# facebook/zstd

Hardware: NVIDIA H100
Metric: compress GB/s (input) at level 1 (higher is better)
Workload: dtype u8

## Files before the change

zstd_b200/csrc/zb_api.cu:

```cuda
#include <cuda_runtime.h>
#include <stdio.h>
#include <stdlib.h>
#include <string.h>
#include <vector>
#include <memory>
#include <mutex>
#include <thread>
#include <new>
#include <time.h>
#include "../../include/zstd_b200.h"
#include "zb_common.h"
#include "zb_kernels.h"

static inline u32 hb32(u32 v) { return 31u - (u32)__builtin_clz(v); }

typedef struct { u32 windowLog, chainLog, hashLog, searchLog, minMatch, targetLength, strategy; } ZbCParams;
struct Row { u8 W, C, H, S, L, TL, strat; };
static const Row kRows[4][5] = {
    { {19,12,13,1,6,1,1}, {19,13,14,1,7,0,1}, {20,15,16,1,6,0,1}, {21,16,17,1,5,0,2}, {21,18,18,1,5,0,2} },
    { {18,12,13,1,5,1,1}, {18,13,14,1,6,0,1}, {18,14,14,1,5,0,2}, {18,16,16,1,4,0,2}, {18,16,16,1,4,0,2} },
    { {17,12,12,1,5,1,1}, {17,12,13,1,6,0,1}, {17,13,15,1,5,0,1}, {17,15,16,2,5,0,2}, {17,17,17,2,4,0,2} },
    { {14,12,13,1,5,1,1}, {14,14,15,1,5,0,1}, {14,14,15,1,4,0,1}, {14,14,15,2,4,0,2}, {14,14,15,2,4,0,2} },
};

// ... 93 lines not shown
        size_t const c = want < 2 * cap ? 2 * cap : want;
        T* q = NULL; bool pin = !pageable;
        if (pin && cudaMallocHost((void**)&q, c * sizeof(T)) != cudaSuccess) { cudaGetLastError(); pin = false; }
        if (!pin) q = (T*)malloc(c * sizeof(T));
        if (n) memcpy(q, p, n * sizeof(T));
        size_t const keep = n;
        release(); p = q; n = keep; cap = c; pinned = pin;
    }
    void push_back(const T& v) { if (n == cap) reserve(cap ? 2 * cap : 64); p[n++] = v; }
    void resize(size_t m) { reserve(m); if (m > n) memset((void*)(p + n), 0, (m - n) * sizeof(T)); n = m; }
    void clear() { n = 0; }
    size_t size() const { return n; }
    T* data() { return p; }
    const T* data() const { return p; }
    T& back() { return p[n - 1]; }
    T& operator[](size_t i) { return p[i]; }
    const T& operator[](size_t i) const { return p[i]; }
};
struct ZbLdmFrame { u32 frame; ZbLdmParams prm; u64 matchBase; u64 prefix; };
struct ZbPlan { ZbVec<ZbBlock> blocks; ZbVec<ZbChunk> chunks; ZbVec<ZbFrame> frames; std::vector<ZbGroup> groups; ZbStrides sd; bool unsupported;
                std::vector<ZbLdmFrame> ldm; u64 ldmMatches;
                u64 frameBytes, frameBlocks; u32 frameMaxBlock;
                void reset() { blocks.clear(); chunks.clear(); frames.clear(); groups.clear(); unsupported = false; ldm.clear(); ldmMatches = 0;
                               frameBytes = frameBlocks = 0; frameMaxBlock = 0; } };

enum { EV_START, EV_K0, EV_K1, EV_K2, EV_K3, EV_MID, EV_KEND, EV_END, EV_PHASES };

struct ZSTD_CCtx_s {
    int device;
    int bindDevice;
    ZbStream stream;
    ZbDevBuf<ZbChunk> d_chunks;
    ZbDevBuf<u8> d_work;
    u32 devWaveBlocks;
    ZbStream waveStream[ZB_WAVE_SLOTS_MAX + 1];
    u32 waveSlots;
    u32 hostWaveSlots;
    u32 hostWaveBlocks;
    ZbDevBuf<ZbBlock> d_blocks; ZbDevBuf<ZbFrame> d_frames;
    ZbDevBuf<u64> d_outOffsets, d_frameSizes;
    ZbDevBuf<u64> d_totals;
    ZbHostBuf<u64> h_totals;
    ZbDevBuf<u8> d_in, d_out;
    std::unique_ptr<ZSTD_CDict, ZbCDictFree> callDict;
    ZbEvents ev;
    ZbEvents evH2D, evStitch, evSize, evD2H;
    ZSTDB200_stats stats;
    int advLevel, advChecksum, advNoDictID;
    int advLdm;
    u32 advLdmPrm[4];
    ZbDevBuf<u64> d_ldmMatch, d_ldmFirst; ZbDevBuf<u32> d_ldmCnt; ZbDevBuf<u8> d_ldmScratch;
    std::unique_ptr<ZSTD_CDict, ZbCDictFree> advLocalDict;
    const ZSTD_CDict* advRefCDict;
    const u8* advPrefix; size_t advPrefixSize; bool advPrefixOnDevice;
    ZbDevBuf<u8> d_prefix;
    ZbPlan plan;
    u8* stIn; size_t stInSize, stInCap;
    u8* stOut; size_t stOutSize, stOutPos, stOutCap;
    int stFrames;
    int advDelims;
    ZbDevBuf<ZSTD_Sequence> d_seqIn;
    ZbDevBuf<u8> d_seqTile, d_seqBlk; ZbDevBuf<u64> d_seqCtrl;
    ZbOrder order; ZbEvents evStage, evJoin;
    ZbPlan asyncPlan;
    ZbHostBuf<u8> stage[ZSTDB200_ASYNC_SLOTS]; bool stageBusy[ZSTDB200_ASYNC_SLOTS]; u32 stageNext;
};
// ... 21 lines not shown
    c->device = -1;
    c->bindDevice = zb_contextDevice();
    c->advLevel = 3;
    c->asyncPlan.blocks.pageable = c->asyncPlan.chunks.pageable = c->asyncPlan.frames.pageable = true;
    {   const char* s = getenv("ZSTDB200_SERIAL"); const char* w = getenv("ZSTDB200_WAVE_BLOCKS");
        c->devWaveBlocks = (s && atoi(s)) ? 0u : (w ? (u32)atoi(w) : 1024u);
        const char* n = getenv("ZSTDB200_WAVE_SLOTS"); const char* h = getenv("ZSTDB200_HOST_WAVE_BLOCKS");
        c->waveSlots = n ? (u32)atoi(n) : ZB_WAVE_SLOTS_DEFAULT;
        c->hostWaveSlots = n ? (u32)atoi(n) : ZB_HOST_WAVE_SLOTS_DEFAULT;
        if (c->waveSlots < 1u) c->waveSlots = 1u;
        if (c->waveSlots > ZB_WAVE_SLOTS_MAX) c->waveSlots = ZB_WAVE_SLOTS_MAX;
        if (c->hostWaveSlots < 1u) c->hostWaveSlots = 1u;
        if (c->hostWaveSlots > ZB_WAVE_SLOTS_MAX) c->hostWaveSlots = ZB_WAVE_SLOTS_MAX;
        c->hostWaveBlocks = (h && atoi(h) > 0) ? (u32)atoi(h) : ZB_HOST_WAVE_BLOCKS; }
    return c;
}

static size_t zb_ctxInit(ZSTD_CCtx* c)
{
    if (c->device >= 0) { CK(cudaSetDevice(c->device)); return 0; }
    int n = 0;
    if (cudaGetDeviceCount(&n) != cudaSuccess || n == 0) { cudaGetLastError(); return ZB_ERR(ZB_error_GENERIC); }
    int dev = c->bindDevice;
    if (dev < 0) { if (cudaGetDevice(&dev) != cudaSuccess) dev = 0; }
    CK(cudaSetDevice(dev));
    ZbStream st; ZbEvents ev, evStage, evJoin; ZbOrder order;
    TRY(st.ensure());
    TRY(ev.ensure(EV_PHASES, true));
    TRY(order.create()); TRY(evStage.ensure(ZSTDB200_ASYNC_SLOTS, false)); TRY(evJoin.ensure(ZB_WAVE_SLOTS_MAX, false));
    static ZbdFseCTable defaults[3]; static std::once_flag once;
    std::call_once(once, [] { zb_buildDefaultTables(defaults); });
    CK(zb_upload_default_tables(defaults, st));
    CK(cudaStreamSynchronize(st));
    c->stream = std::move(st); c->ev = std::move(ev);
    c->order = std::move(order); c->evStage = std::move(evStage); c->evJoin = std::move(evJoin);
    c->device = dev;
    return 0;
}

extern "C" size_t ZSTD_freeCCtx(ZSTD_CCtx* c)
{
    if (!c) return 0;
    free(c->stIn); free(c->stOut);
    return zb_deleteOnDevice(c, &c->order);
}

static size_t zb_ensureDesc(ZSTD_CCtx* c, size_t nbBlocks, size_t nbFrames, size_t nbWaves, size_t nbChunks)
{
    TRY(c->d_chunks.ensure(nbChunks));
    TRY(c->d_blocks.ensure(nbBlocks)); TRY(c->d_outOffsets.ensure(nbBlocks + 1));
    TRY(c->d_frames.ensure(nbFrames)); TRY(c->d_frameSizes.ensure(nbFrames));
    TRY(c->d_totals.ensure(nbWaves)); TRY(c->h_totals.ensure(nbWaves));
    return 0;
}

struct ZbCall {
    void* dst; size_t dstCapacity; const void* src;
    const size_t* frameOffsets; const size_t* frameSizes; size_t nbFrames;
    const ZSTD_CDict* cdict;
    int level; size_t* cSizes;
    bool deviceMemory; cudaStream_t stream;
    bool checksum, noDictID;
    u64 partBegin = 0, partEnd = ~0ull;
    const u32* ldm = nullptr;
    const u8* prefix = nullptr; u64 prefixSize = 0; bool prefixOnDevice = false;
    unsigned long long* result = nullptr; unsigned long long* d_cSizes = nullptr;
// ... 171 lines not shown
    }
    size_t const nbBlocks = P.blocks.size();
    TRY(c->d_ldmMatch.ensure(P.ldmMatches));
    TRY(c->d_ldmFirst.ensure(nbBlocks));
    TRY(c->d_ldmCnt.ensure(nbBlocks));
    TRY(c->d_ldmScratch.ensure(scratch));
    return 0;
}
static size_t zb_runLdm(ZSTD_CCtx* c, const ZbPlan& P, const u8* d_src, const u8* d_prefix, cudaStream_t stream, unsigned* launches)
{
    for (size_t i = 0; i < P.ldm.size(); i++) {
        ZbLdmFrame const& lf = P.ldm[i];
        ZbFrame const& fr = P.frames[lf.frame];
        CK(zb_launch_ldm(d_prefix, lf.prefix, d_src + fr.srcOff, fr.srcSize, &lf.prm, c->d_ldmScratch, fr.nbBlocks, lf.matchBase, c->d_ldmMatch,
                         c->d_ldmFirst + fr.firstBlock, c->d_ldmCnt + fr.firstBlock, stream));
        *launches += 4u + 3u * ((lf.prm.hashLog - lf.prm.bucketSizeLog + 7u) / 8u);
        if (lf.prefix >= lf.prm.minMatch && fr.srcSize >= lf.prm.minMatch) *launches += 1u;
    }
    return 0;
}

static size_t zb_runBlocks(ZSTD_CCtx* c, const ZbPlan& P, const u8* d_src, const u8* d_dictEnd, const ZbDictEntropy* d_de, u32 b0, u32 b1, u32 c0, u32 c1,
                           const ZbWorkRows& rows, cudaStream_t stream, bool timed, unsigned* launches)
{
    for (int phase = 0; phase < 3; phase++) {
        for (size_t g = 0; g < P.groups.size(); g++) {
            ZbGroup const& G = P.groups[g];
            u32 const lo = G.b0 > b0 ? G.b0 : b0, hi = G.b1 < b1 ? G.b1 : b1;
            u32 const clo = G.c0 > c0 ? G.c0 : c0, chi = G.c1 < c1 ? G.c1 : c1;
            if (lo >= hi) continue;
            ZbWorkRows const R = rows.at(lo - b0);
            if (phase == 0) {
                ZbLdmView lv; lv.match = c->d_ldmMatch; lv.first = c->d_ldmFirst + lo; lv.cnt = c->d_ldmCnt + lo;
                CK(zb_launch_match(d_src, d_dictEnd, d_dictEnd ? G.image : (const u32*)0, c->d_blocks + lo, hi - lo, c->d_chunks + clo, chi - clo, lo, &G.prm, &R,
                                   (timed && P.groups.size() == 1) ? c->ev[EV_MID] : (cudaEvent_t)0, stream, G.ldm ? &lv : nullptr));
                *launches += G.prm.strategy == 2 ? 4 : 3;
            } else if (phase == 1) {
                CK(zb_launch_literals(c->d_blocks + lo, hi - lo, &G.prm, &R.sd, d_de, R.lits, R.body, R.meta, stream));
                *launches += 1;
            } else {
                CK(zb_launch_sequences(d_src, c->d_blocks + lo, hi - lo, &G.prm, &R.sd, d_de, R.seqs, R.dist, R.body, R.meta, stream));
                *launches += 1;
            }
        }
        if (timed) CK(cudaEventRecord(c->ev[EV_K1 + phase], stream));
    }
    return 0;
}

static u64 zb_xxh64(const u8* p, size_t len)
{
    u64 const P1 = 0x9E3779B185EBCA87ull, P2 = 0xC2B2AE3D27D4EB4Full, P3 = 0x165667B19E3779F9ull, P4 = 0x85EBCA77C2B2AE63ull, P5 = 0x27D4EB2F165667C5ull;
    auto rotl = [](u64 x, int r) { return (x << r) | (x >> (64 - r)); };
    auto rd64 = [](const u8* q) { u64 v; memcpy(&v, q, 8); return v; };
    auto rd32 = [](const u8* q) { u32 v; memcpy(&v, q, 4); return v; };
    auto round = [&](u64 acc, u64 in) { return rotl(acc + in * P2, 31) * P1; };
    auto merge = [&](u64 acc, u64 v) { return (acc ^ round(0, v)) * P1 + P4; };
    const u8* const end = p + len;
    u64 h;
    if (len >= 32) {
        u64 v1 = P1 + P2, v2 = P2, v3 = 0, v4 = 0 - P1;
        const u8* const limit = end - 32;
        do { v1 = round(v1, rd64(p)); v2 = round(v2, rd64(p + 8)); v3 = round(v3, rd64(p + 16)); v4 = round(v4, rd64(p + 24)); p += 32; } while (p <= limit);
        h = rotl(v1, 1) + rotl(v2, 7) + rotl(v3, 12) + rotl(v4, 18);
        h = merge(h, v1); h = merge(h, v2); h = merge(h, v3); h = merge(h, v4);
    } else h = P5;
    h += (u64)len;
// ... 906 lines not shown
```

zstd_b200/csrc/zb_common.h:

```cpp
#ifndef ZB_COMMON_H
#define ZB_COMMON_H
#include <stdint.h>
#include <stddef.h>

typedef uint8_t  u8;
typedef uint16_t u16;
typedef uint32_t u32;
typedef uint64_t u64;

#define ZB_BLOCK_MAX     (128u << 10)
#define ZB_PRIME_BYTES   (128u << 10)
#define ZB_CHUNK_BLOCKS  4u
#define ZB_BATCH         1024u
#define ZB_TAG_BITS      11u
#define ZB_FAST_HASHLOG_MAX   14u
#ifndef ZB_DFAST_SHORT_MAX
#define ZB_DFAST_SHORT_MAX    28672u
#endif
#ifndef ZB_DFAST_LONGLOG_MAX
#define ZB_DFAST_LONGLOG_MAX  14u
#endif
#define ZB_FAR           0xFFFFu

#define ZB_BT_RAW 0
// ... 164 lines not shown

static inline bool zb_isErr(size_t c) { return c > ZB_ERR(ZB_error_maxCode); }

#define CK(x) do { cudaError_t e_ = (x); if (e_ != cudaSuccess) { \
    if (getenv("ZSTDB200_DEBUG")) fprintf(stderr, "zstd_b200: CUDA error %s at %s:%d\n", cudaGetErrorString(e_), __FILE__, __LINE__); \
    cudaGetLastError(); return ZB_ERR(e_ == cudaErrorMemoryAllocation ? ZB_error_memory_allocation : ZB_error_GENERIC); } } while (0)
#define TRY(x) do { size_t const e_ = (x); if (zb_isErr(e_)) return e_; } while (0)

inline thread_local bool zb_noAlloc = false;

template <typename T, bool Pinned> struct ZbBuf {
    T* p = nullptr; size_t cap = 0;
    ZbBuf() = default;
    ZbBuf(const ZbBuf&) = delete; ZbBuf& operator=(const ZbBuf&) = delete;
    ~ZbBuf() { release(); }
    void release() { if (p) { if (Pinned) cudaFreeHost(p); else cudaFree(p); } p = nullptr; cap = 0; }
    size_t ensure(size_t need, size_t headroom = 0) {
        if (need <= cap) return 0;
        if (zb_noAlloc) return ZB_ERR(ZB_error_stage_wrong);
        release();
        size_t const bytes = (need + headroom) * sizeof(T);
        CK(Pinned ? cudaMallocHost((void**)&p, bytes) : cudaMalloc((void**)&p, bytes));
        cap = need + headroom;
        return 0;
    }
    operator T*() const { return p; }
};
template <typename T> using ZbDevBuf = ZbBuf<T, false>;
template <typename T> using ZbHostBuf = ZbBuf<T, true>;

enum ZbWorkKind { ZB_WORK_FAST, ZB_WORK_DFAST, ZB_WORK_SEQUENCES };
struct ZbWorkRows {
    ZbStrides sd;
    ZbBlockMeta* meta; u64* seqs; u8* lits; u8* body; u16* dist; u32* far; u16* dist2; u32* far2; ZbSegMeta* segmeta;
    ZbWorkRows at(size_t row) const {
        ZbWorkRows r = *this;
        auto down = [row](auto*& p, size_t stride) { if (p) p += row * stride; };
        down(r.meta, 1); down(r.seqs, sd.seq); down(r.lits, sd.lit); down(r.body, sd.body);
        down(r.dist, sd.dist); down(r.far, sd.dist); down(r.dist2, sd.dist); down(r.far2, sd.dist); down(r.segmeta, zb_segsPerRow(sd));
        return r;
    }
};
static inline size_t zb_workLayout(u8* base, size_t rows, ZbWorkKind kind, const ZbStrides& sd, ZbWorkRows* out)
{
    bool const match = kind != ZB_WORK_SEQUENCES;
    if (3ull * sd.state > sd.dist) return ZB_ERR(ZB_error_GENERIC);
    if (match && ((u64)sd.seq * 8u > (u64)sd.dist * 4u || ((u64)sd.seq + 1u) * 4u > (u64)sd.dist * 2u)) return ZB_ERR(ZB_error_GENERIC);
    ZbWorkRows w = {};
    w.sd = sd;
    size_t const align = (size_t)2 << 20;
    size_t bytes = 0;
    auto place = [&](auto*& p, size_t n) {
        if (base) p = reinterpret_cast<std::remove_reference_t<decltype(p)>>(base + bytes);
        bytes = (bytes + n * sizeof(*p) + 256u + align - 1u) & ~(align - 1u);
    };
    place(w.meta, rows); place(w.seqs, rows * sd.seq); place(w.lits, rows * sd.lit); place(w.body, rows * sd.body);
    place(w.dist, rows * sd.dist);
    if (match) { place(w.far, rows * sd.dist); place(w.segmeta, rows * zb_segsPerRow(sd)); }
    if (kind == ZB_WORK_DFAST) { place(w.dist2, rows * sd.dist); place(w.far2, rows * sd.dist); }
    if (base) *out = w;
    return bytes;
}

struct ZbStream {
    cudaStream_t s = nullptr;
    ZbStream() = default;
    ZbStream& operator=(ZbStream&& o) { std::swap(s, o.s); return *this; }
    ~ZbStream() { if (s) cudaStreamDestroy(s); }
    size_t ensure() {
        if (s) return 0;
        if (zb_noAlloc) return ZB_ERR(ZB_error_stage_wrong);
        CK(cudaStreamCreateWithFlags(&s, cudaStreamNonBlocking));
        return 0;
    }
    operator cudaStream_t() const { return s; }
};

struct ZbEvents {
    std::vector<cudaEvent_t> ev; bool timed = false;
    ZbEvents() = default;
    ZbEvents& operator=(ZbEvents&& o) { ev.swap(o.ev); std::swap(timed, o.timed); return *this; }
    ~ZbEvents() { release(); }
    void release() { for (cudaEvent_t e : ev) cudaEventDestroy(e); ev.clear(); }
    size_t ensure(size_t n, bool timing) {
        if (n <= ev.size() && timing == timed) return 0;
        if (zb_noAlloc) return ZB_ERR(ZB_error_stage_wrong);
        release();
        timed = timing;
        while (ev.size() < n) {
            cudaEvent_t e;
            CK(cudaEventCreateWithFlags(&e, timing ? cudaEventDefault : cudaEventDisableTiming));
// ... 54 lines not shown
```

zstd_b200/csrc/zb_kernels.h:

```cpp
#ifndef ZB_KERNELS_H
#define ZB_KERNELS_H
#include <cuda_runtime.h>
#include "zb_common.h"

#ifdef __cplusplus
extern "C" {
#endif

cudaError_t zb_launch_dict_image(const u8* d_dictEnd, const ZbChunk* d_dictChunk, const ZbParams* prm, u32* d_image, cudaStream_t stream);
cudaError_t zb_launch_match(const u8* d_src, const u8* d_dictEnd, const u32* d_image, const ZbBlock* d_blocks, u32 nbBlocks,
                            const ZbChunk* d_chunks, u32 nbChunks, u32 slotFirstBlock, const ZbParams* prm, const ZbWorkRows* rows,
                            cudaEvent_t evMid, cudaStream_t stream, const ZbLdmView* ldm = nullptr);

size_t zb_ldm_scratch_bytes(u64 P, u64 n, const ZbLdmParams* prm);
cudaError_t zb_launch_ldm(const u8* d_prefix, u64 P, const u8* d_frame, u64 n, const ZbLdmParams* prm, void* d_scratch, u32 nbBlocks,
                          u64 matchBase, u64* d_match, u64* d_ldmFirst, u32* d_ldmCnt, cudaStream_t stream);

cudaError_t zb_launch_seq_partition(const void* d_seqs, u32 n, int expl, u64* d_tileLen, u32* d_tileEnds, u64* d_ctrl, cudaStream_t stream);
cudaError_t zb_launch_seq_place(const void* d_seqs, u32 n, int expl, const u64* d_tileLen, const u32* d_tileEnds,
                                u64 srcSize, u64 window, u64 dictContent, u32 blockMax, u32 nbBlocks,
                                u64* d_blockEnd, u32* d_blockSeq, u32* d_blockFirst, u64* d_blockFirstPos, u64* d_ctrl, cudaStream_t stream);
cudaError_t zb_launch_seq_blocks(const u64* d_blockEnd, const u32* d_blockSeq, u32 nbBlocks, u32 blockMax, u32 dictFlag,
                                 ZbBlock* d_blocks, u32* d_blockFirst, u64* d_blockFirstPos, u64* d_ctrl, cudaStream_t stream);
cudaError_t zb_launch_seq_convert(const u8* d_src, const ZbBlock* d_blocks, u32 nbBlocks, const u32* d_blockFirst, const u64* d_blockFirstPos,
                                  const void* d_seqs, u32 n, const ZbParams* prm, const ZbWorkRows* rows, cudaStream_t stream);

void zb_buildDefaultTables(ZbdFseCTable* out3);
cudaError_t zb_upload_default_tables(const ZbdFseCTable* host3, cudaStream_t stream);

size_t zb_loadDictionary(ZbDictEntropy* de, const u8* dict, size_t dictSize);

cudaError_t zb_launch_literals(const ZbBlock* d_blocks, u32 nbBlocks, const ZbParams* prm, const ZbStrides* sd, const ZbDictEntropy* d_de,
                               const u8* d_lits, u8* d_body, ZbBlockMeta* d_meta, cudaStream_t stream);

cudaError_t zb_launch_sequences(const u8* d_src, const ZbBlock* d_blocks, u32 nbBlocks, const ZbParams* prm, const ZbStrides* sd, const ZbDictEntropy* d_de,
                                const u64* d_seqs, u16* d_stateBits, u8* d_body, ZbBlockMeta* d_meta, cudaStream_t stream);

cudaError_t zb_launch_stitch(const u8* d_src, const ZbBlock* d_blocks, u32 nbBlocks, const ZbFrame* d_frames, const ZbWorkRows* rows,
                             u64* d_outOffsets, const u64* d_base, u64* d_total,
                             u8* d_dst, u64 dstCapacity, cudaStream_t stream);
cudaError_t zb_launch_checksums(const u8* d_src, const ZbFrame* d_frames, u32 nbFrames, const u64* d_outOffsets, u8* d_dst, u64 dstCapacity, cudaStream_t stream);
cudaError_t zb_launch_frame_sizes(const ZbFrame* d_frames, u32 nbFrames, const u64* d_outOffsets,
                                  u64* d_frameSizes, cudaStream_t stream);
cudaError_t zb_launch_call_result(const ZbFrame* d_frames, u32 nbFrames, const u64* d_outOffsets, const u64* d_total,
                                  u64 dstCapacity, unsigned long long* d_cSizes, unsigned long long* d_result, cudaStream_t stream);
// ... 6 lines not shown
```

zstd_b200/csrc/zb_match.cu:

```cuda
#include "zb_device.cuh"
#include "zb_kernels.h"
#include "zb_merge.cuh"

template <bool DICT>
__device__ __forceinline__ u32 zb_count_fwd(const ZbSeg& sg, u32 a, u32 offset, u32 be, u32 lane)
{
    u32 fwd = 0;
    while (true) {
        u32 const pa = a + fwd + 8u * lane;
        u32 m;
        if (pa + 8u <= be) {
            u64 const x = zb_seg_ld64x<DICT>(sg, pa) ^ zb_seg_ld64x<DICT>(sg, pa - offset);
            m = x ? (u32)((__ffsll((long long)x) - 1) >> 3) : 8u;
        } else {
            m = 0;
            while (pa + m < be && zb_seg_byte<DICT>(sg, pa + m) == zb_seg_byte<DICT>(sg, pa + m - offset)) m++;
        }
        u32 const inc = __ballot_sync(ZB_FULL, m != 8u);
        if (inc == 0) { fwd += 256u; continue; }
        int const f = __ffs((int)inc) - 1;
        fwd += 8u * (u32)f + __shfl_sync(ZB_FULL, m, f);
        return fwd;
    }
}
// ... 229 lines not shown
        u32 const pat = zb_walk_pattern_res<P>(step == insStep ? r0 : zb_walk_residue(xa - shift, step), step);
        bool const output = !buildImage && x0 >= H + shift;
        u32 const qb0 = x0 - shift - H;
        size_t const row = output ? (size_t)(cd.firstBlock - slotFirstBlock + (qb0 >> cd.blockLog)) * sd.dist + (qb0 & blockMask) : 0;
        if (zb_walk_batch<MLS, P, true>(table, xa, cur, pat, N, shift, D, total, xLow, xEnd, fbase, dbase, output, distT + row, farT + row)) li = x0 + ZB_BATCH;
        r0 += stepInc; if (r0 >= insStep) r0 -= insStep;
        x0 += ZB_BATCH;
    };
    while (x0 < xEnd) {
        if (WALK_STEADY && x0 >= xIntLoB && x0 + 4u * ZB_BATCH <= xIntHi) {
            if (D != 0u && li < D + shift) li = D + shift;
            do { steadyBatch(rawA, shA); steadyBatch(rawB, shB); } while (x0 + 4u * ZB_BATCH <= xIntHi);
        }
        doBatch(rawA, shA);
        if (x0 >= xEnd) break;
        doBatch(rawB, shB);
    }
    if (buildImage) { __syncthreads(); for (u32 i = t; i < N; i += THREADS) imageOut[i] = table[i]; }
}

#ifndef PARSE_WARPS
#define PARSE_WARPS 8
#endif
#ifndef PARSE_MIN_CTAS
#define PARSE_MIN_CTAS 6
#endif
__device__ __forceinline__ u32 zb_dist_at(const u16* __restrict__ d16, const u32* __restrict__ far, u32 i)
{
    u32 const d = d16[i];
    return d == ZB_FAR ? far[i] : d;
}

template <bool DICT>
__global__ void __launch_bounds__(32 * PARSE_WARPS, DICT ? (40 / PARSE_WARPS) : PARSE_MIN_CTAS)
zb_parse_kernel(const u8* __restrict__ src, const u8* __restrict__ dictEnd, const ZbBlock* __restrict__ blocks, u32 nbBlocks, ZbParams prm, ZbStrides sd,
                const u16* __restrict__ dist, const u32* __restrict__ far, u64* __restrict__ seqs, ZbBlockMeta* __restrict__ meta, ZbSegMeta* __restrict__ segmeta)
{
    u32 const lane = threadIdx.x & 31u;
    u32 const g = blockIdx.x * PARSE_WARPS + (threadIdx.x >> 5);
    u32 const segs = zb_segsPerRow(sd);
    u32 const b = g / segs, k = g % segs;
    if (b >= nbBlocks) return;
    ZbBlock const bd = blocks[b];
    const u16* const mydist = dist + (size_t)b * sd.dist;
    const u32* const myfar = far + (size_t)b * sd.dist;
    const u8* const base = src + bd.srcOff - bd.histLen;
    u32 const bs = bd.histLen, blockEnd = bd.histLen + bd.size;
    ZbSeg sg; sg.hi = base; sg.lo = base; sg.split = 0;
    if (DICT && (bd.flags & ZB_FLAG_DICT)) { sg.lo = dictEnd - bd.dictLen; sg.split = bd.dictLen; }

    if (bd.size < 7u) {
        if (lane == 0 && k == 0) {
            ZbBlockMeta m; m.nbSeq = 0; m.litSize = bd.size; m.litSecSize = 0; m.bodySize = bd.size;
            m.type = ZB_BT_RAW; m.forceRaw = 1; m.rleByte = 0; m.pad = 0;
            meta[b] = m;
        }
        return;
    }
    u32 const ss = bs + k * ZB_PARSE_SEG;
    if (ss >= blockEnd) {
        if (lane == 0) { ZbSegMeta z; z.nbSeq = 0; z.pad[0] = z.pad[1] = z.pad[2] = 0; segmeta[(size_t)b * segs + k] = z; }
        return;
    }
    u32 const se = min(ss + ZB_PARSE_SEG, blockEnd);
    u32 const be = blockEnd;

    u32 ip = ss, anchor = ss;
    u32 rep1 = 0, rep2 = 0, nbSeq = 0;
    if ((bd.flags & ZB_FLAG_FIRST) && k == 0u) { rep1 = prm.startRep[0]; rep2 = prm.startRep[1]; }

    auto ld4 = [&](u32 x) { return DICT ? (u32)zb_seg_ld64x<DICT>(sg, x) : zb_ld32w2(sg.hi + x); };
    while (ip < se && ip + 8u <= be) {
        u32 const step = prm.stepSize + ((ip - anchor) >> 7);
        u32 const p = ip + (lane >> 1) * step + (lane & 1u);
        bool const act = (p < se) && (p + 8u <= be);
// ... 22 lines not shown
                if (probe < offset) { tent &= tent - 1u; continue; }
            }
            u32 const a = (wtype == 1u) ? probe : probe + 4u;
            u32 const kb = lane + 1u;
            bool const bIn = (probe >= anchor + kb) && (probe >= offset + kb);
            u32 const b0 = bIn ? zb_seg_byte<DICT>(sg, probe - kb) : 0u;
            u32 const b1 = bIn ? zb_seg_byte<DICT>(sg, probe - offset - kb) : 0u;
            u32 const pa = a + 8u * lane;
            u32 const q = min(pa, be - 8u);
            u64 const xf = zb_seg_ld64x<DICT>(sg, q) ^ zb_seg_ld64x<DICT>(sg, q - offset);
            u64 const xs = xf >> (8u * min(pa - q, 7u));
            u32 m = xs ? (u32)((__ffsll((long long)xs) - 1) >> 3) : 8u;
            m = pa >= be ? 0u : min(m, be - pa);
            u32 const okb = __ballot_sync(ZB_FULL, bIn && b0 == b1);
            u32 const inc = __ballot_sync(ZB_FULL, m != 8u);
            u32 fwd;
            if (inc == 0u) fwd = 256u + zb_count_fwd<DICT>(sg, a + 256u, offset, be, lane);
            else { int const f = __ffs((int)inc) - 1; fwd = 8u * (u32)f + __shfl_sync(ZB_FULL, m, f); }
            if (wtype == 1u && fwd < 4u) { tent &= tent - 1u; continue; }
            fwdFrom4 = (wtype == 1u) ? fwd - 4u : fwd;
            back = (okb == ZB_FULL) ? 32u + zb_back_coop<DICT>(sg, probe - 32u, offset, anchor, lane) : (u32)(__ffs((int)~okb) - 1);
            found = true;
            break;
        }
        if (!found) { ip += 16u * step; continue; }
        u32 const ms = probe - back;
        u32 const mlen = back + 4u + fwdFrom4;
        if (wtype == 3u) { u32 const t = rep2; rep2 = rep1; rep1 = t; }
        else if (wtype == 1u) { rep2 = rep1; rep1 = offset; }
        if (lane == 0) seqs[(size_t)b * sd.seq + k * (ZB_PARSE_SEG / 4u) + nbSeq] = zb_pack_raw(offset, mlen, ms - bs);
        nbSeq++;
        ip = ms + mlen; anchor = ip;
    }
    if (lane == 0) { ZbSegMeta z; z.nbSeq = nbSeq; z.pad[0] = z.pad[1] = z.pad[2] = 0; segmeta[blockIdx.x * PARSE_WARPS + (threadIdx.x >> 5)] = z; }
}

template <bool DICT>
__global__ void __launch_bounds__(32 * PARSE_WARPS)
zb_parse_dfast_kernel(const u8* __restrict__ src, const u8* __restrict__ dictEnd, const ZbBlock* __restrict__ blocks, u32 nbBlocks, ZbParams prm, ZbStrides sd,
                      const u16* __restrict__ distLong, const u32* __restrict__ farLong, const u16* __restrict__ distShort, const u32* __restrict__ farShort,
                      u64* __restrict__ seqs, ZbBlockMeta* __restrict__ meta, ZbSegMeta* __restrict__ segmeta)
{
    u32 const lane = threadIdx.x & 31u;
    u32 const g = blockIdx.x * PARSE_WARPS + (threadIdx.x >> 5);
    u32 const segs = zb_segsPerRow(sd);
    u32 const b = g / segs, k = g % segs;
    if (b >= nbBlocks) return;
    ZbBlock const bd = blocks[b];
    u64* const myseq = seqs + (size_t)b * sd.seq + (size_t)k * (ZB_PARSE_SEG / 4u);
    const u16* const dLp = distLong + (size_t)b * sd.dist;
    const u32* const fLp = farLong + (size_t)b * sd.dist;
    const u16* const dSp = distShort + (size_t)b * sd.dist;
    const u32* const fSp = farShort + (size_t)b * sd.dist;
    const u8* const base = src + bd.srcOff - bd.histLen;
    u32 const bs = bd.histLen, blockEnd = bd.histLen + bd.size;
    ZbSeg sg; sg.hi = base; sg.lo = base; sg.split = 0;
    if (DICT && (bd.flags & ZB_FLAG_DICT)) { sg.lo = dictEnd - bd.dictLen; sg.split = bd.dictLen; }

    if (bd.size < 7u) {
        if (lane == 0 && k == 0) {
            ZbBlockMeta m; m.nbSeq = 0; m.litSize = bd.size; m.litSecSize = 0; m.bodySize = bd.size;
            m.type = ZB_BT_RAW; m.forceRaw = 1; m.rleByte = 0; m.pad = 0;
            meta[b] = m;
        }
        return;
    }
    u32 const ss = bs + k * ZB_PARSE_SEG;
    if (ss >= blockEnd) {
        if (lane == 0) { ZbSegMeta z; z.nbSeq = 0; z.pad[0] = z.pad[1] = z.pad[2] = 0; segmeta[(size_t)b * segs + k] = z; }
        return;
    }
    u32 const se = min(ss + ZB_PARSE_SEG, blockEnd);
    u32 const be = blockEnd;
    u32 ip = ss, anchor = ss, searchStart = ss;
    u32 rep1 = 0, rep2 = 0, nbSeq = 0;
    if ((bd.flags & ZB_FLAG_FIRST) && k == 0u) { rep1 = prm.startRep[0]; rep2 = prm.startRep[1]; }

    while (ip < se && ip + 9u <= be) {
        u32 const step = 1u + ((ip - searchStart) >> 8);
        u32 const p = ip + lane * step;
// ... 24 lines not shown
            if (wtype == 3u) { ms = probe; offset = rep2; mlen = 4u + zb_count_fwd<DICT>(sg, probe + 4u, rep2, be, lane); found = true; break; }
            if (wtype == 2u) { ms = probe + 1u; offset = rep1; mlen = 4u + zb_count_fwd<DICT>(sg, probe + 5u, rep1, be, lane); found = true; break; }
            if (wtype == 1u) {
                u32 const f0 = zb_count_fwd<DICT>(sg, probe, wL, be, lane);
                if (f0 >= 8u) {
                    u32 const back = zb_back_coop<DICT>(sg, probe, wL, anchor, lane);
                    ms = probe - back; offset = wL; mlen = back + f0; found = true; break;
                }
                if (lane == (u32)winner) hit = dS ? 4u : 0u;
                if (wS == 0u) { tent &= ~(1u << winner); }
                continue;
            }
            {   u32 const f0 = zb_count_fwd<DICT>(sg, probe, wS, be, lane);
                if (f0 < 4u) { tent &= ~(1u << winner); if (lane == (u32)winner) hit = 0u; continue; }
                u32 mp = probe, mo = wS, ml = f0;
                if (wL1) {
                    u32 const f1 = zb_count_fwd<DICT>(sg, probe + 1u, wL1, be, lane);
                    if (f1 >= 8u && f1 > ml) { mp = probe + 1u; mo = wL1; ml = f1; }
                }
                u32 const back = zb_back_coop<DICT>(sg, mp, mo, anchor, lane);
                ms = mp - back; offset = mo; mlen = back + ml; wtype = 1u; found = true; break;
            }
        }
        if (!found) { ip += 32u * step; continue; }
        if (wtype == 3u) { u32 const t = rep2; rep2 = rep1; rep1 = t; }
        else if (wtype == 1u) { rep2 = rep1; rep1 = offset; }
        if (lane == 0) myseq[nbSeq] = zb_pack_raw(offset, mlen, ms - bs);
        nbSeq++;
        ip = ms + mlen; anchor = ip; searchStart = ip;
    }
    if (lane == 0) { ZbSegMeta z; z.nbSeq = nbSeq; z.pad[0] = z.pad[1] = z.pad[2] = 0; segmeta[(size_t)b * segs + k] = z; }
}

struct ZbRepHist { u32 r1, r2, r3; };
__device__ __forceinline__ u32 zb_rep_code(ZbRepHist& h, u32 off, u32 ll)
{
    u32 code;
    if (ll > 0u) {
        if (off == h.r1) return 1u;
        if (off == h.r2) { code = 2u; h.r2 = h.r1; h.r1 = off; return code; }
        if (off == h.r3) { code = 3u; h.r3 = h.r2; h.r2 = h.r1; h.r1 = off; return code; }
    } else {
        if (off == h.r2) { code = 1u; h.r2 = h.r1; h.r1 = off; return code; }
        if (off == h.r3) { code = 2u; h.r3 = h.r2; h.r2 = h.r1; h.r1 = off; return code; }
        if (h.r1 > 1u && off == h.r1 - 1u) { code = 3u; h.r3 = h.r2; h.r2 = h.r1; h.r1 = off; return code; }
    }
    h.r3 = h.r2; h.r2 = h.r1; h.r1 = off;
    return off + 3u;
}

#ifndef MERGE_MIN_CTAS
#define MERGE_MIN_CTAS 6
#endif
#define SEG_SLOTS (ZB_PARSE_SEG / 4u)

__device__ __forceinline__ u32 zb_block_excl(bool flag, u32* wsum, u32* total)
{
    u32 const lane = threadIdx.x & 31u, warp = threadIdx.x >> 5;
    u32 const bal = __ballot_sync(ZB_FULL, flag);
    if (lane == 0u) wsum[warp] = __popc(bal);
    __syncthreads();
    u32 before = __popc(bal & ((1u << lane) - 1u)), t = 0;
    for (u32 w = 0; w < MERGE_THREADS / 32u; w++) { if (w < warp) before += wsum[w]; t += wsum[w]; }
    __syncthreads();
    *total = t;
    return before;
// ... 205 lines not shown
    zb_walk_kernel<MLS, P><<<nbChunks, ZB_BATCH / P, (size_t)N * 4u, stream>>>(d_src, d_dictEnd, d_chunks, insStep, N, sd, slotFirstBlock, d_dist, d_far, d_imageIn, d_imageOut);
    return cudaGetLastError();
}
template <int MLS>
static cudaError_t zb_launch_walk_m(const u8* d_src, const u8* d_dictEnd, const ZbChunk* d_chunks, u32 nbChunks, u32 N, u32 insStep, const ZbStrides& sd,
                                    u32 slotFirstBlock, u16* d_dist, u32* d_far, const u32* d_imageIn, u32* d_imageOut, cudaStream_t stream)
{
    size_t const smem = (size_t)N * 4u;
    if (smem <= 56u * 1024u)  return zb_launch_walk_p<MLS, WALK_P_SMALL>(d_src, d_dictEnd, d_chunks, nbChunks, N, insStep, sd, slotFirstBlock, d_dist, d_far, d_imageIn, d_imageOut, stream);
    if (smem <= 113u * 1024u) return zb_launch_walk_p<MLS, WALK_P_MID>(d_src, d_dictEnd, d_chunks, nbChunks, N, insStep, sd, slotFirstBlock, d_dist, d_far, d_imageIn, d_imageOut, stream);
    return zb_launch_walk_p<MLS, 1>(d_src, d_dictEnd, d_chunks, nbChunks, N, insStep, sd, slotFirstBlock, d_dist, d_far, d_imageIn, d_imageOut, stream);
}
static cudaError_t zb_launch_walk(const u8* d_src, const u8* d_dictEnd, const ZbChunk* d_chunks, u32 nbChunks, u32 mls, u32 N, u32 insStep, const ZbStrides& sd,
                                  u32 slotFirstBlock, u16* d_dist, u32* d_far, const u32* d_imageIn, u32* d_imageOut, cudaStream_t stream)
{
    switch (mls) {
    case 4: return zb_launch_walk_m<4>(d_src, d_dictEnd, d_chunks, nbChunks, N, insStep, sd, slotFirstBlock, d_dist, d_far, d_imageIn, d_imageOut, stream);
    case 5: return zb_launch_walk_m<5>(d_src, d_dictEnd, d_chunks, nbChunks, N, insStep, sd, slotFirstBlock, d_dist, d_far, d_imageIn, d_imageOut, stream);
    case 6: return zb_launch_walk_m<6>(d_src, d_dictEnd, d_chunks, nbChunks, N, insStep, sd, slotFirstBlock, d_dist, d_far, d_imageIn, d_imageOut, stream);
    case 7: return zb_launch_walk_m<7>(d_src, d_dictEnd, d_chunks, nbChunks, N, insStep, sd, slotFirstBlock, d_dist, d_far, d_imageIn, d_imageOut, stream);
    default: return zb_launch_walk_m<8>(d_src, d_dictEnd, d_chunks, nbChunks, N, insStep, sd, slotFirstBlock, d_dist, d_far, d_imageIn, d_imageOut, stream);
    }
}

extern "C" cudaError_t zb_launch_dict_image(const u8* d_dictEnd, const ZbChunk* d_dictChunk, const ZbParams* prm, u32* d_image, cudaStream_t stream)
{
    ZbStrides const sd = zb_strides(ZB_BLOCK_MAX);
    cudaError_t e = zb_launch_walk(nullptr, d_dictEnd, d_dictChunk, 1, prm->mls, prm->tableN, prm->insStep, sd, 0, nullptr, nullptr, nullptr, d_image, stream);
    if (e == cudaSuccess && prm->strategy == 2)
        e = zb_launch_walk(nullptr, d_dictEnd, d_dictChunk, 1, 8, prm->tableNLong, prm->insStep, sd, 0, nullptr, nullptr, nullptr, d_image + prm->tableN, stream);
    return e;
}

extern "C" cudaError_t zb_launch_match(const u8* d_src, const u8* d_dictEnd, const u32* d_image, const ZbBlock* d_blocks, u32 nbBlocks,
                                       const ZbChunk* d_chunks, u32 nbChunks, u32 slotFirstBlock, const ZbParams* prm, const ZbWorkRows* rows,
                                       cudaEvent_t evMid, cudaStream_t stream, const ZbLdmView* ldm)
{
    if (nbBlocks == 0) return cudaSuccess;
    ZbStrides const sd = rows->sd;
    u16* const d_dist = rows->dist; u32* const d_far = rows->far; u16* const d_dist2 = rows->dist2; u32* const d_far2 = rows->far2;
    u64* const d_seqs = rows->seqs; u8* const d_lits = rows->lits; ZbBlockMeta* const d_meta = rows->meta; ZbSegMeta* const d_segmeta = rows->segmeta;
    cudaError_t e;
    u32 const segs = zb_segsPerRow(sd);
    u32 const sgrid = (u32)(((u64)nbBlocks * segs + PARSE_WARPS - 1) / PARSE_WARPS);
    if (prm->strategy == 2) {
        e = zb_launch_walk(d_src, d_dictEnd, d_chunks, nbChunks, 8, prm->tableNLong, prm->insStep, sd, slotFirstBlock, d_dist, d_far, d_image ? d_image + prm->tableN : nullptr, nullptr, stream); if (e != cudaSuccess) return e;
        e = zb_launch_walk(d_src, d_dictEnd, d_chunks, nbChunks, prm->mls, prm->tableN, prm->insStep, sd, slotFirstBlock, d_dist2, d_far2, d_image, nullptr, stream); if (e != cudaSuccess) return e;
        if (evMid) cudaEventRecord(evMid, stream);
        if (d_dictEnd) zb_parse_dfast_kernel<true><<<sgrid, 32 * PARSE_WARPS, 0, stream>>>(d_src, d_dictEnd, d_blocks, nbBlocks, *prm, sd, d_dist, d_far, d_dist2, d_far2, d_seqs, d_meta, d_segmeta);
        else           zb_parse_dfast_kernel<false><<<sgrid, 32 * PARSE_WARPS, 0, stream>>>(d_src, nullptr, d_blocks, nbBlocks, *prm, sd, d_dist, d_far, d_dist2, d_far2, d_seqs, d_meta, d_segmeta);
    } else {
        e = zb_launch_walk(d_src, d_dictEnd, d_chunks, nbChunks, prm->mls, prm->tableN, prm->insStep, sd, slotFirstBlock, d_dist, d_far, d_image, nullptr, stream); if (e != cudaSuccess) return e;
        if (evMid) cudaEventRecord(evMid, stream);
        if (d_dictEnd) zb_parse_kernel<true><<<sgrid, 32 * PARSE_WARPS, 0, stream>>>(d_src, d_dictEnd, d_blocks, nbBlocks, *prm, sd, d_dist, d_far, d_seqs, d_meta, d_segmeta);
        else           zb_parse_kernel<false><<<sgrid, 32 * PARSE_WARPS, 0, stream>>>(d_src, nullptr, d_blocks, nbBlocks, *prm, sd, d_dist, d_far, d_seqs, d_meta, d_segmeta);
    }
    if (segs == 1u && sd.dist <= 8192u)
        zb_merge_small_kernel<<<(nbBlocks + MERGE_THREADS / 32u - 1u) / (MERGE_THREADS / 32u), MERGE_THREADS, 0, stream>>>(d_src, d_blocks, nbBlocks, *prm, sd, d_segmeta, d_seqs, d_lits, d_meta);
    else if (ldm)
        zb_merge_segments_kernel<true><<<nbBlocks, MERGE_THREADS, 0, stream>>>(d_src, d_blocks, *prm, sd, d_segmeta, d_seqs, d_lits, d_meta, *ldm, d_far, d_dist);
    else
        zb_merge_segments_kernel<false><<<nbBlocks, MERGE_THREADS, 0, stream>>>(d_src, d_blocks, *prm, sd, d_segmeta, d_seqs, d_lits, d_meta, ZbLdmView(), nullptr, nullptr);
    return cudaGetLastError();
}
```

Measured before the change: 103.0.

## Use persistent parse kernels with atomic dynamic segment claiming

Parse kernels become persistent. The grid is sized to occupancy times SM count, and each warp claims segments through an atomic counter that is reset by a memset before each launch. This is meant to balance uneven per-segment parse work and cut tail imbalance and block-scheduling overhead. It adds an extra memset launch, one atomic per segment, and a claim slot in the workspace, plus optional clock-instrumentation code.

```diff
diff --git a/zstd_b200/csrc/zb_api.cu b/zstd_b200/csrc/zb_api.cu
--- a/zstd_b200/csrc/zb_api.cu
+++ b/zstd_b200/csrc/zb_api.cu
@@ -149,6 +149,7 @@
     ZbStream stream;
     ZbDevBuf<ZbChunk> d_chunks;
     ZbDevBuf<u8> d_work;
+    u32 parseGrid[4];
     u32 devWaveBlocks;
     ZbStream waveStream[ZB_WAVE_SLOTS_MAX + 1];
     u32 waveSlots;
@@ -236,6 +237,7 @@
     std::call_once(once, [] { zb_buildDefaultTables(defaults); });
     CK(zb_upload_default_tables(defaults, st));
     CK(cudaStreamSynchronize(st));
+    CK(zb_parse_grids(c->parseGrid));
     c->stream = std::move(st); c->ev = std::move(ev);
     c->order = std::move(order); c->evStage = std::move(evStage); c->evJoin = std::move(evJoin);
     c->device = dev;
@@ -473,7 +475,7 @@
             ZbWorkRows const R = rows.at(lo - b0);
             if (phase == 0) {
                 ZbLdmView lv; lv.match = c->d_ldmMatch; lv.first = c->d_ldmFirst + lo; lv.cnt = c->d_ldmCnt + lo;
-                CK(zb_launch_match(d_src, d_dictEnd, d_dictEnd ? G.image : (const u32*)0, c->d_blocks + lo, hi - lo, c->d_chunks + clo, chi - clo, lo, &G.prm, &R,
+                CK(zb_launch_match(d_src, d_dictEnd, d_dictEnd ? G.image : (const u32*)0, c->d_blocks + lo, hi - lo, c->d_chunks + clo, chi - clo, lo, &G.prm, &R, c->parseGrid,
                                    (timed && P.groups.size() == 1) ? c->ev[EV_MID] : (cudaEvent_t)0, stream, G.ldm ? &lv : nullptr));
                 *launches += G.prm.strategy == 2 ? 4 : 3;
             } else if (phase == 1) {
diff --git a/zstd_b200/csrc/zb_common.h b/zstd_b200/csrc/zb_common.h
--- a/zstd_b200/csrc/zb_common.h
+++ b/zstd_b200/csrc/zb_common.h
@@ -220,12 +220,12 @@
 enum ZbWorkKind { ZB_WORK_FAST, ZB_WORK_DFAST, ZB_WORK_SEQUENCES };
 struct ZbWorkRows {
     ZbStrides sd;
-    ZbBlockMeta* meta; u64* seqs; u8* lits; u8* body; u16* dist; u32* far; u16* dist2; u32* far2; ZbSegMeta* segmeta;
+    ZbBlockMeta* meta; u64* seqs; u8* lits; u8* body; u16* dist; u32* far; u16* dist2; u32* far2; ZbSegMeta* segmeta; u32* claim;
     ZbWorkRows at(size_t row) const {
         ZbWorkRows r = *this;
         auto down = [row](auto*& p, size_t stride) { if (p) p += row * stride; };
         down(r.meta, 1); down(r.seqs, sd.seq); down(r.lits, sd.lit); down(r.body, sd.body);
-        down(r.dist, sd.dist); down(r.far, sd.dist); down(r.dist2, sd.dist); down(r.far2, sd.dist); down(r.segmeta, zb_segsPerRow(sd));
+        down(r.dist, sd.dist); down(r.far, sd.dist); down(r.dist2, sd.dist); down(r.far2, sd.dist); down(r.segmeta, zb_segsPerRow(sd)); down(r.claim, 1);
         return r;
     }
 };
@@ -244,7 +244,7 @@
     };
     place(w.meta, rows); place(w.seqs, rows * sd.seq); place(w.lits, rows * sd.lit); place(w.body, rows * sd.body);
     place(w.dist, rows * sd.dist);
-    if (match) { place(w.far, rows * sd.dist); place(w.segmeta, rows * zb_segsPerRow(sd)); }
+    if (match) { place(w.far, rows * sd.dist); place(w.segmeta, rows * zb_segsPerRow(sd)); place(w.claim, rows); }
     if (kind == ZB_WORK_DFAST) { place(w.dist2, rows * sd.dist); place(w.far2, rows * sd.dist); }
     if (base) *out = w;
     return bytes;
diff --git a/zstd_b200/csrc/zb_kernels.h b/zstd_b200/csrc/zb_kernels.h
--- a/zstd_b200/csrc/zb_kernels.h
+++ b/zstd_b200/csrc/zb_kernels.h
@@ -10,7 +10,8 @@
 cudaError_t zb_launch_dict_image(const u8* d_dictEnd, const ZbChunk* d_dictChunk, const ZbParams* prm, u32* d_image, cudaStream_t stream);
 cudaError_t zb_launch_match(const u8* d_src, const u8* d_dictEnd, const u32* d_image, const ZbBlock* d_blocks, u32 nbBlocks,
                             const ZbChunk* d_chunks, u32 nbChunks, u32 slotFirstBlock, const ZbParams* prm, const ZbWorkRows* rows,
-                            cudaEvent_t evMid, cudaStream_t stream, const ZbLdmView* ldm = nullptr);
+                            const u32* parseGrid, cudaEvent_t evMid, cudaStream_t stream, const ZbLdmView* ldm = nullptr);
+cudaError_t zb_parse_grids(u32 grid[4]);
 
 size_t zb_ldm_scratch_bytes(u64 P, u64 n, const ZbLdmParams* prm);
 cudaError_t zb_launch_ldm(const u8* d_prefix, u64 P, const u8* d_frame, u64 n, const ZbLdmParams* prm, void* d_scratch, u32 nbBlocks,
diff --git a/zstd_b200/csrc/zb_match.cu b/zstd_b200/csrc/zb_match.cu
--- a/zstd_b200/csrc/zb_match.cu
+++ b/zstd_b200/csrc/zb_match.cu
@@ -285,15 +285,12 @@
 }
 
 template <bool DICT>
-__global__ void __launch_bounds__(32 * PARSE_WARPS, DICT ? (40 / PARSE_WARPS) : PARSE_MIN_CTAS)
-zb_parse_kernel(const u8* __restrict__ src, const u8* __restrict__ dictEnd, const ZbBlock* __restrict__ blocks, u32 nbBlocks, ZbParams prm, ZbStrides sd,
-                const u16* __restrict__ dist, const u32* __restrict__ far, u64* __restrict__ seqs, ZbBlockMeta* __restrict__ meta, ZbSegMeta* __restrict__ segmeta)
-{
-    u32 const lane = threadIdx.x & 31u;
-    u32 const g = blockIdx.x * PARSE_WARPS + (threadIdx.x >> 5);
+__device__ __forceinline__ void zb_parse_segment(u32 g, u32 lane, const u8* __restrict__ src, const u8* __restrict__ dictEnd, const ZbBlock* __restrict__ blocks,
+                                                 const ZbParams& prm, const ZbStrides& sd, const u16* __restrict__ dist, const u32* __restrict__ far,
+                                                 u64* __restrict__ seqs, ZbBlockMeta* __restrict__ meta, ZbSegMeta* __restrict__ segmeta)
+{
     u32 const segs = zb_segsPerRow(sd);
     u32 const b = g / segs, k = g % segs;
-    if (b >= nbBlocks) return;
     ZbBlock const bd = blocks[b];
     const u16* const mydist = dist + (size_t)b * sd.dist;
     const u32* const myfar = far + (size_t)b * sd.dist;
@@ -382,20 +379,17 @@
         nbSeq++;
         ip = ms + mlen; anchor = ip;
     }
-    if (lane == 0) { ZbSegMeta z; z.nbSeq = nbSeq; z.pad[0] = z.pad[1] = z.pad[2] = 0; segmeta[blockIdx.x * PARSE_WARPS + (threadIdx.x >> 5)] = z; }
+    if (lane == 0) { ZbSegMeta z; z.nbSeq = nbSeq; z.pad[0] = z.pad[1] = z.pad[2] = 0; segmeta[(size_t)b * segs + k] = z; }
 }
 
 template <bool DICT>
-__global__ void __launch_bounds__(32 * PARSE_WARPS)
-zb_parse_dfast_kernel(const u8* __restrict__ src, const u8* __restrict__ dictEnd, const ZbBlock* __restrict__ blocks, u32 nbBlocks, ZbParams prm, ZbStrides sd,
-                      const u16* __restrict__ distLong, const u32* __restrict__ farLong, const u16* __restrict__ distShort, const u32* __restrict__ farShort,
-                      u64* __restrict__ seqs, ZbBlockMeta* __restrict__ meta, ZbSegMeta* __restrict__ segmeta)
-{
-    u32 const lane = threadIdx.x & 31u;
-    u32 const g = blockIdx.x * PARSE_WARPS + (threadIdx.x >> 5);
+__device__ __forceinline__ void zb_parse_dfast_segment(u32 g, u32 lane, const u8* __restrict__ src, const u8* __restrict__ dictEnd, const ZbBlock* __restrict__ blocks,
+                                                       const ZbParams& prm, const ZbStrides& sd,
+                                                       const u16* __restrict__ distLong, const u32* __restrict__ farLong, const u16* __restrict__ distShort, const u32* __restrict__ farShort,
+                                                       u64* __restrict__ seqs, ZbBlockMeta* __restrict__ meta, ZbSegMeta* __restrict__ segmeta)
+{
     u32 const segs = zb_segsPerRow(sd);
     u32 const b = g / segs, k = g % segs;
-    if (b >= nbBlocks) return;
     ZbBlock const bd = blocks[b];
     u64* const myseq = seqs + (size_t)b * sd.seq + (size_t)k * (ZB_PARSE_SEG / 4u);
     const u16* const dLp = distLong + (size_t)b * sd.dist;
@@ -486,6 +480,72 @@
     if (lane == 0) { ZbSegMeta z; z.nbSeq = nbSeq; z.pad[0] = z.pad[1] = z.pad[2] = 0; segmeta[(size_t)b * segs + k] = z; }
 }
 
+#ifndef PARSE_STATIC
+#define PARSE_STATIC 0
+#endif
+__device__ __forceinline__ u32 zb_parse_claim(u32* claim, u32 lane)
+{
+    u32 g = 0;
+    if (lane == 0u) g = atomicAdd(claim, 1u);
+    return __shfl_sync(ZB_FULL, g, 0);
+}
+#ifdef PARSE_CLOCKS
+struct ZbParseClock { u64 c0, c1, t0, t1; u32 sm, cta, warp, pad; };
+#define ZB_PARSE_CLOCK_MAX (1u << 20)
+__device__ ZbParseClock zb_parseClock[ZB_PARSE_CLOCK_MAX];
+__device__ __forceinline__ u64 zb_globaltimer() { u64 t; asm volatile("mov.u64 %0, %%globaltimer;" : "=l"(t)); return t; }
+__device__ __forceinline__ u32 zb_smid() { u32 s; asm volatile("mov.u32 %0, %%smid;" : "=r"(s)); return s; }
+#define ZB_PARSE_CLOCK_START u64 const c0_ = clock64(), t0_ = zb_globaltimer();
+#define ZB_PARSE_CLOCK_END(g) if (lane == 0u && (g) < ZB_PARSE_CLOCK_MAX) { \
+    ZbParseClock r_; r_.c0 = c0_; r_.c1 = clock64(); r_.t0 = t0_; r_.t1 = zb_globaltimer(); r_.sm = zb_smid(); r_.cta = blockIdx.x; \
+    r_.warp = threadIdx.x >> 5; r_.pad = 0; zb_parseClock[g] = r_; }
+extern "C" __attribute__((visibility("default"))) int ZSTDB200_parseClocks(void* dst, unsigned n)
+{
+    if (n > ZB_PARSE_CLOCK_MAX) n = ZB_PARSE_CLOCK_MAX;
+    if (cudaDeviceSynchronize() != cudaSuccess || cudaMemcpyFromSymbol(dst, zb_parseClock, (size_t)n * sizeof(ZbParseClock)) != cudaSuccess) return -1;
+    return (int)sizeof(ZbParseClock);
+}
+#else
+#define ZB_PARSE_CLOCK_START
+#define ZB_PARSE_CLOCK_END(g)
+#endif
+
+template <bool DICT>
+__global__ void __launch_bounds__(32 * PARSE_WARPS, DICT ? (40 / PARSE_WARPS) : PARSE_MIN_CTAS)
+zb_parse_kernel(const u8* __restrict__ src, const u8* __restrict__ dictEnd, const ZbBlock* __restrict__ blocks, u32 nbBlocks, ZbParams prm, ZbStrides sd,
+                const u16* __restrict__ dist, const u32* __restrict__ far, u64* __restrict__ seqs, ZbBlockMeta* __restrict__ meta, ZbSegMeta* __restrict__ segmeta,
+                u32* __restrict__ claim)
+{
+    u32 const lane = threadIdx.x & 31u;
+    u32 const nSeg = nbBlocks * zb_segsPerRow(sd);
+    u32 g = PARSE_STATIC ? blockIdx.x * PARSE_WARPS + (threadIdx.x >> 5) : zb_parse_claim(claim, lane);
+    while (g < nSeg) {
+        ZB_PARSE_CLOCK_START
+        zb_parse_segment<DICT>(g, lane, src, dictEnd, blocks, prm, sd, dist, far, seqs, meta, segmeta);
+        ZB_PARSE_CLOCK_END(g)
+        if (PARSE_STATIC) break;
+        g = zb_parse_claim(claim, lane);
+    }
+}
+
+template <bool DICT>
+__global__ void __launch_bounds__(32 * PARSE_WARPS)
+zb_parse_dfast_kernel(const u8* __restrict__ src, const u8* __restrict__ dictEnd, const ZbBlock* __restrict__ blocks, u32 nbBlocks, ZbParams prm, ZbStrides sd,
+                      const u16* __restrict__ distLong, const u32* __restrict__ farLong, const u16* __restrict__ distShort, const u32* __restrict__ farShort,
+                      u64* __restrict__ seqs, ZbBlockMeta* __restrict__ meta, ZbSegMeta* __restrict__ segmeta, u32* __restrict__ claim)
+{
+    u32 const lane = threadIdx.x & 31u;
+    u32 const nSeg = nbBlocks * zb_segsPerRow(sd);
+    u32 g = PARSE_STATIC ? blockIdx.x * PARSE_WARPS + (threadIdx.x >> 5) : zb_parse_claim(claim, lane);
+    while (g < nSeg) {
+        ZB_PARSE_CLOCK_START
+        zb_parse_dfast_segment<DICT>(g, lane, src, dictEnd, blocks, prm, sd, distLong, farLong, distShort, farShort, seqs, meta, segmeta);
+        ZB_PARSE_CLOCK_END(g)
+        if (PARSE_STATIC) break;
+        g = zb_parse_claim(claim, lane);
+    }
+}
+
 struct ZbRepHist { u32 r1, r2, r3; };
 __device__ __forceinline__ u32 zb_rep_code(ZbRepHist& h, u32 off, u32 ll)
 {
@@ -757,9 +817,22 @@
     return e;
 }
 
+extern "C" cudaError_t zb_parse_grids(u32 grid[4])
+{
+    int dev = 0, sms = 0, per[4] = { 0, 0, 0, 0 };
+    cudaError_t e = cudaGetDevice(&dev);
+    if (e == cudaSuccess) e = cudaDeviceGetAttribute(&sms, cudaDevAttrMultiProcessorCount, dev);
+    if (e == cudaSuccess) e = cudaOccupancyMaxActiveBlocksPerMultiprocessor(&per[0], zb_parse_kernel<false>, 32 * PARSE_WARPS, 0);
+    if (e == cudaSuccess) e = cudaOccupancyMaxActiveBlocksPerMultiprocessor(&per[1], zb_parse_kernel<true>, 32 * PARSE_WARPS, 0);
+    if (e == cudaSuccess) e = cudaOccupancyMaxActiveBlocksPerMultiprocessor(&per[2], zb_parse_dfast_kernel<false>, 32 * PARSE_WARPS, 0);
+    if (e == cudaSuccess) e = cudaOccupancyMaxActiveBlocksPerMultiprocessor(&per[3], zb_parse_dfast_kernel<true>, 32 * PARSE_WARPS, 0);
+    for (int k = 0; k < 4; k++) grid[k] = (u32)(per[k] > 0 ? per[k] : 1) * (u32)(sms > 0 ? sms : 1);
+    return e;
+}
+
 extern "C" cudaError_t zb_launch_match(const u8* d_src, const u8* d_dictEnd, const u32* d_image, const ZbBlock* d_blocks, u32 nbBlocks,
                                        const ZbChunk* d_chunks, u32 nbChunks, u32 slotFirstBlock, const ZbParams* prm, const ZbWorkRows* rows,
-                                       cudaEvent_t evMid, cudaStream_t stream, const ZbLdmView* ldm)
+                                       const u32* parseGrid, cudaEvent_t evMid, cudaStream_t stream, const ZbLdmView* ldm)
 {
     if (nbBlocks == 0) return cudaSuccess;
     ZbStrides const sd = rows->sd;
@@ -768,17 +841,21 @@
     cudaError_t e;
     u32 const segs = zb_segsPerRow(sd);
     u32 const sgrid = (u32)(((u64)nbBlocks * segs + PARSE_WARPS - 1) / PARSE_WARPS);
+    int const pv = (prm->strategy == 2 ? 2 : 0) + (d_dictEnd ? 1 : 0);
+    u32 const pgrid = (PARSE_STATIC || sgrid < parseGrid[pv]) ? sgrid : parseGrid[pv];
     if (prm->strategy == 2) {
         e = zb_launch_walk(d_src, d_dictEnd, d_chunks, nbChunks, 8, prm->tableNLong, prm->insStep, sd, slotFirstBlock, d_dist, d_far, d_image ? d_image + prm->tableN : nullptr, nullptr, stream); if (e != cudaSuccess) return e;
         e = zb_launch_walk(d_src, d_dictEnd, d_chunks, nbChunks, prm->mls, prm->tableN, prm->insStep, sd, slotFirstBlock, d_dist2, d_far2, d_image, nullptr, stream); if (e != cudaSuccess) return e;
         if (evMid) cudaEventRecord(evMid, stream);
-        if (d_dictEnd) zb_parse_dfast_kernel<true><<<sgrid, 32 * PARSE_WARPS, 0, stream>>>(d_src, d_dictEnd, d_blocks, nbBlocks, *prm, sd, d_dist, d_far, d_dist2, d_far2, d_seqs, d_meta, d_segmeta);
-        else           zb_parse_dfast_kernel<false><<<sgrid, 32 * PARSE_WARPS, 0, stream>>>(d_src, nullptr, d_blocks, nbBlocks, *prm, sd, d_dist, d_far, d_dist2, d_far2, d_seqs, d_meta, d_segmeta);
+        e = cudaMemsetAsync(rows->claim, 0, sizeof(u32), stream); if (e != cudaSuccess) return e;
+        if (d_dictEnd) zb_parse_dfast_kernel<true><<<pgrid, 32 * PARSE_WARPS, 0, stream>>>(d_src, d_dictEnd, d_blocks, nbBlocks, *prm, sd, d_dist, d_far, d_dist2, d_far2, d_seqs, d_meta, d_segmeta, rows->claim);
+        else           zb_parse_dfast_kernel<false><<<pgrid, 32 * PARSE_WARPS, 0, stream>>>(d_src, nullptr, d_blocks, nbBlocks, *prm, sd, d_dist, d_far, d_dist2, d_far2, d_seqs, d_meta, d_segmeta, rows->claim);
     } else {
         e = zb_launch_walk(d_src, d_dictEnd, d_chunks, nbChunks, prm->mls, prm->tableN, prm->insStep, sd, slotFirstBlock, d_dist, d_far, d_image, nullptr, stream); if (e != cudaSuccess) return e;
         if (evMid) cudaEventRecord(evMid, stream);
-        if (d_dictEnd) zb_parse_kernel<true><<<sgrid, 32 * PARSE_WARPS, 0, stream>>>(d_src, d_dictEnd, d_blocks, nbBlocks, *prm, sd, d_dist, d_far, d_seqs, d_meta, d_segmeta);
-        else           zb_parse_kernel<false><<<sgrid, 32 * PARSE_WARPS, 0, stream>>>(d_src, nullptr, d_blocks, nbBlocks, *prm, sd, d_dist, d_far, d_seqs, d_meta, d_segmeta);
+        e = cudaMemsetAsync(rows->claim, 0, sizeof(u32), stream); if (e != cudaSuccess) return e;
+        if (d_dictEnd) zb_parse_kernel<true><<<pgrid, 32 * PARSE_WARPS, 0, stream>>>(d_src, d_dictEnd, d_blocks, nbBlocks, *prm, sd, d_dist, d_far, d_seqs, d_meta, d_segmeta, rows->claim);
+        else           zb_parse_kernel<false><<<pgrid, 32 * PARSE_WARPS, 0, stream>>>(d_src, nullptr, d_blocks, nbBlocks, *prm, sd, d_dist, d_far, d_seqs, d_meta, d_segmeta, rows->claim);
     }
     if (segs == 1u && sd.dist <= 8192u)
         zb_merge_small_kernel<<<(nbBlocks + MERGE_THREADS / 32u - 1u) / (MERGE_THREADS / 32u), MERGE_THREADS, 0, stream>>>(d_src, d_blocks, nbBlocks, *prm, sd, d_segmeta, d_seqs, d_lits, d_meta);
```

After: 105.8, median of 6. +2.7%, better.
